# Hydrology-IFH/roger

Hardware: AMD Instinct MI355X
Metric: cell-timesteps/sec on SVAT_benchmark grid (higher is better)
Workload: dtype f64

## Files before the change

roger_amd/build.py:

```python
import os
import subprocess
import sys

PKG = os.path.dirname(os.path.abspath(__file__))
REPO = os.path.dirname(PKG)
CSRC = os.path.join(PKG, "csrc")
LIB = os.path.join(PKG, "libroger_hip.so")
HIPCC = os.environ.get("HIPCC", "/opt/rocm/bin/hipcc")

FLAGS = ["--offload-arch=gfx950", "-O3", "-std=c++17", "-fPIC", "-ffp-contract=off",
         "-I" + os.path.join(REPO, "include"), "-I" + CSRC]


_SAS_DEPS = ("rh_sas_dev.h", "rh_sas_tables.inc", "include/roger_hip_sas.h", "include/rh_sas_arrays.def", "include/roger_hip.h")
UNITS = {
    "roger_hip": ("rh_host.h", "rh_physics.h", "rh_pow.h", "rh_col.h", "rh_sets.inc", "include/roger_hip.h", "include/rh_fields.def",
                  "rh_dev_state.h", "rh_control.h", "rh_step.h", "rh_routing.h", "rh_routing_host.h", "rh_rccl.h"),
    "rh_sas": _SAS_DEPS + ("rh_host.h",),
    "rh_sas_det_iso": _SAS_DEPS + ("rh_sas_kernels.h",),
    "rh_sas_det_anion": _SAS_DEPS + ("rh_sas_kernels.h",),
    "rh_sas_euler_iso": _SAS_DEPS + ("rh_sas_solvers_impl.h",),
    "rh_sas_euler_anion": _SAS_DEPS + ("rh_sas_solvers_impl.h",),
    "rh_sas_rk4_iso": _SAS_DEPS + ("rh_sas_solvers_impl.h",),
    "rh_sas_rk4_anion": _SAS_DEPS + ("rh_sas_solvers_impl.h",),
}
OBJ = os.path.join(PKG, "_obj")


def _newer(target, sources):
    if not os.path.exists(target):
        return True
    t = os.path.getmtime(target)
    return any(os.path.getmtime(s) > t for s in sources)


def _dep_path(d):
    return os.path.join(REPO, d) if d.startswith("include/") else os.path.join(CSRC, d)


def build_native(force=False, verbose=False):
    subprocess.run([sys.executable, os.path.join(REPO, "tools", "gen_sets.py")], check=True)
    os.makedirs(OBJ, exist_ok=True)
    this = os.path.abspath(__file__)
    jobs, objs = [], []
    for unit, deps in UNITS.items():
        src, obj = os.path.join(CSRC, unit + ".hip"), os.path.join(OBJ, unit + ".o")
        objs.append(obj)
        if force or _newer(obj, [src, this] + [_dep_path(d) for d in deps]):
            cmd = [HIPCC] + FLAGS + ["-c", src, "-o", obj]
            if verbose:
                print(" ".join(cmd))
            jobs.append((cmd, subprocess.Popen(cmd)))
    for cmd, job in jobs:
        if job.wait() != 0:
            raise subprocess.CalledProcessError(job.returncode, cmd)
    if force or jobs or _newer(LIB, objs):
        cmd = [HIPCC, "--offload-arch=gfx950", "-shared", "-fPIC"] + objs + ["-o", LIB]
        if verbose:
            print(" ".join(cmd))
        subprocess.run(cmd, check=True)
    return LIB


if __name__ == "__main__":
    print(build_native(force="--force" in sys.argv, verbose=True))
```

roger_amd/csrc/rh_dev_state.h:

```cpp
#ifndef RH_DEV_STATE_H
#define RH_DEV_STATE_H

#define RH_BLOCK 256
#ifndef RH_STRIDE_PAD
#define RH_STRIDE_PAD 0
#endif
#define RH_PRED_BLOCKS 1024
#define RH_DONE_GROUPS 256
#define RH_DONE_STRIDE 32
#define RH_DEVERR_FORCING 1u
#define RH_TAIL_USE_NEXT 1
#define RH_TAIL_CTRL 2
#define RH_TAIL_HOOKS 4
#define RH_TAIL_PRE 16
#define RH_TAIL_SKIP 8
#define RH_SRC_WORD3 0
#ifndef RH_WSTRIDE
#define RH_WSTRIDE 16
#endif
#define RH_SRC_SUMW 1
#ifndef RH_STEP_WAVES
#define RH_STEP_WAVES 2
#endif

struct DevState {
    Consts K;
    rh_scalars S;
    StepCtx X;
    unsigned long long words[4];
    unsigned long long bflags[2][RH_PRED_BLOCKS];
    unsigned long long day_bflags[RH_PRED_BLOCKS];
    int pred_blocks;
    unsigned long long sumw[64 * RH_WSTRIDE];
    unsigned int done_grp[RH_DONE_GROUPS * RH_DONE_STRIDE];
    unsigned int done_top;
    unsigned long long sanity_last;
    unsigned long long pre_words[64];
    int day_cache_ok, day_cache_pad;
    unsigned long long day_fb;
    double day_agg[3];
    unsigned int err_flags;
    rh_scalars S_next;
    StepCtx X_next;
    double *diag;
    long long *diag_steps;
    long long diag_interval;
    int diag_rate, diag_collect, diag_slots;
    int diag_planes[32];
    unsigned long long keep[(RH_NPLANES + 63) / 64];
    int keep_any;
    int *dt_log;
    int dt_log_cap, dt_log_n;
    double forc[3][RH_SLOTS_PER_DAY];
    const double *forc_cell[3];
    double *agg_cell;
    unsigned long long frontw[64 * RH_WSTRIDE], dayw[64 * RH_WSTRIDE], day_word;
    int per_cell;
    const double *series[3];
    const int64_t *calendar[3];
    int64_t nitt_forc;
    long long t_end;
    int skipped;
    int monthly;
    const double *weights[3];
    int n_stations;
    const int *station_idx;
    double *forc_multi;

    const unsigned long long *pmask;

    const double *mlms;
    int64_t mlms_rows;
    int max_slope_per;
    Luts L;
};

struct HostExport {
    rh_scalars S;
    unsigned long long bad, bad_last;
    unsigned int err, pad;
    unsigned long long seq;
};
// ... 163 lines not shown
```

roger_amd/csrc/rh_step.h:

```cpp
#ifndef RH_STEP_H
#define RH_STEP_H

#define LD(name) rh_ld(a, RH_P_##name, i, c.name);
#define ST(name) rh_st(a, RH_P_##name, i, c.name);

constexpr int rh_param_bit(int plane) {
    switch (plane) {
#define RH_PB(name, bit) case RH_P_##name: return bit;
        RH_PARAM_BITS(RH_PB)
#undef RH_PB
        default: return -1;
    }
}
constexpr bool rh_param_derived(int plane) {
    switch (plane) {
#define RH_PD(name) case RH_P_##name:
        RH_DERIVED_FIELDS(RH_PD)
#undef RH_PD
        return true;
        default: return false;
    }
}
#if defined(RH_CENSUS)
#ifndef RH_CENSUS_PMASK
// ... 71 lines not shown
        RH_SEQ_##seq##_LLOAD_##rt(LDP) RH_SEQ_##seq##_ALIAS_##rt(AL) \
    } else {                                                       \
        RH_SEQ_##seq##_LOAD_##rt(LD)                               \
    }
#define RH_DERIVE(rt)                        \
    if constexpr (LAZY) {                    \
        if (um >> 63) rd_##rt(c, K);         \
        rl_##rt(c, K);                       \
    }
#ifdef RH_CENSUS
#define STK(name)
#else
#define STK(name) \
    if ((keepw[RH_P_##name >> 6] >> (RH_P_##name & 63)) & 1ull) rh_st(a, RH_P_##name, i, c.name);
#endif
#define RH_STORES(seq, rt)                                               \
    if constexpr (LAZY && SPARSE) {                                      \
        RH_SEQ_##seq##_SSTORE_##rt(ST)                                   \
        if constexpr (KEEP) { RH_SEQ_##seq##_KSTORE_##rt(STK) }          \
    } else if constexpr (LAZY) {                                         \
        RH_SEQ_##seq##_LSTORE_##rt(ST)                                   \
    } else {                                                             \
        RH_SEQ_##seq##_STORE_##rt(ST) RH_SEQ_##seq##_ROT_##rt(ROT)       \
    }
#define RH_PIN __builtin_amdgcn_sched_barrier(0);
#ifdef RH_STEP_PHASES
__device__ unsigned long long g_step_phases[256 * 64];
#define RH_PH(k)                                                                          \
    if ((threadIdx.x & 63) == 0) {                                                        \
        const unsigned long long t_ = clock64();                                          \
        atomicAdd(&g_step_phases[(blockIdx.x & 255) * 64 + ph_cls * 20 + (k)], t_ - ph_t);                          \
        ph_t = t_;                                                                        \
    }
#else
#define RH_PH(k)
#endif
#define RH_STEP_BODY(seq, mon_rt, MON_LOADS, MON_RUN, sub_rt, sub_call, ne_rt, ne_call, at_rt, at_call) \
    RH_LOADS(seq, rt_select_prec) RH_LOADS(seq, rt_select_pet) MON_LOADS RH_LOADS(seq, rt_interception) RH_PIN  \
    rt_select_prec(c, X, prec_s, ta_s); RH_STORES(seq, rt_select_prec)                                                \
    rt_select_pet(c, X, pet_v, ta_v); RH_STORES(seq, rt_select_pet) RH_PH(1)                                      \
    q = summary_bits_pt(c.prec, c.ta, K);                                                                \
    MON_RUN                                                                                              \
    RH_LOADS(seq, rt_evapotranspiration) RH_PIN                                                                 \
    rt_interception(c, K); RH_STORES(seq, rt_interception) RH_PH(2)                                               \
    RH_LOADS(seq, rt_snow) RH_PIN                                                                               \
    RH_DERIVE(rt_evapotranspiration) rt_evapotranspiration(c, K); RH_STORES(seq, rt_evapotranspiration) RH_PH(3)  \
    RH_LOADS(seq, rt_inf_events) RH_PIN                                                                         \
    rt_snow(c, K, X); RH_STORES(seq, rt_snow) RH_PH(4)                                                            \
    q = summary_bits_sw(q, c.swe, c.swe_top); if (post) post_summary(D, q, dep);                         \
    RH_LOADS(seq, rt_inf_matrix) RH_PIN                                                                         \
    rt_inf_events(c, K, X); RH_STORES(seq, rt_inf_events) RH_PH(5)                                                \
    RH_LOADS(seq, rt_inf_macropores) RH_PIN                                                                     \
    RH_DERIVE(rt_inf_matrix) rt_inf_matrix(c, K, X); RH_STORES(seq, rt_inf_matrix) RH_PH(6)                       \
    RH_LOADS(seq, rt_inf_cracks) RH_PIN                                                                         \
    RH_DERIVE(rt_inf_macropores) rt_inf_macropores(c, K, X); RH_STORES(seq, rt_inf_macropores) RH_PH(7)           \
    RH_LOADS(seq, rt_inf_finish) RH_PIN                                                                         \
    rt_inf_cracks(c, K, X); RH_STORES(seq, rt_inf_cracks) RH_PH(8)                                                \
    RH_LOADS(seq, sub_rt) RH_PIN                                                                                \
    rt_inf_finish(c, K, X); RH_STORES(seq, rt_inf_finish) RH_PH(9)                                                \
    RH_LOADS(seq, rt_capillary_rise) RH_PIN                                                                     \
    RH_DERIVE(sub_rt) sub_call; RH_STORES(seq, sub_rt) RH_PH(10)                                                   \
    RH_LOADS(seq, rt_storage) RH_PIN                                                                            \
    rt_capillary_rise(c, X); RH_STORES(seq, rt_capillary_rise) RH_PH(11)                                           \
    RH_LOADS(seq, ne_rt) RH_PIN                                                                                 \
    RH_DERIVE(rt_storage) rt_storage(c, X); RH_STORES(seq, rt_storage) RH_PH(12)                                   \
    RH_LOADS(seq, at_rt) RH_PIN                                                                                 \
    bad = ne_call; RH_STORES(seq, ne_rt) RH_PH(13)                                                                 \
    at_call; RH_STORES(seq, at_rt) RH_PH(14)

RH_DEV void post_summary(DevState *D, unsigned long long q, unsigned &dep) {
    unsigned long long qq = 0;
#pragma unroll
    for (int b = 0; b <= QB_P_NE0; ++b) qq |= __ballot((q >> b) & 1ull) ? (1ull << b) : 0ull;
    if ((threadIdx.x & 63) == 0 && qq) {
        const unsigned long long old = __hip_atomic_fetch_or(&D->sumw[(blockIdx.x & 63) * RH_WSTRIDE], qq, __ATOMIC_RELAXED, __HIP_MEMORY_SCOPE_AGENT);
        dep |= (unsigned)(old >> 63);
    }
}

template <bool MONTHLY, bool LATERAL, bool LAZY, bool SPARSE, bool KEEP = false, bool MK1 = false>
RH_DEV void step_column(const Arena &a, DevState *D, const StepCtx *Xp, int64_t i, unsigned long long &q, bool &bad, unsigned &dep, unsigned long long um,
                        bool post) {
    {
    const Consts K = D->K;
    const StepCtx X = *Xp;
    Col c;
    double pet_v = X.pet_sel_w, ta_v = X.ta_sel_w;
    double prec_s = X.prec_sel, ta_s = X.ta_sel;
    unsigned long long keepw[(RH_NPLANES + 63) / 64];
#pragma unroll
    for (int k = 0; k < (RH_NPLANES + 63) / 64; ++k) keepw[k] = KEEP ? D->keep[k] : 0ull;
#ifdef RH_STEP_PHASES
    const int ph_cls = X.dt < 0.5 ? 0 : (X.dt < 12 ? 1 : 2);
    unsigned long long ph_t = clock64();
    if ((threadIdx.x & 63) == 0) atomicAdd(&g_step_phases[(blockIdx.x & 255) * 64 + ph_cls * 20 + 19], 1ull);
#endif
#ifndef RH_CENSUS
    if (D->per_cell && X.sel_w >= 0) {
        pet_v = cell_agg(D, a.n, i, 3 * X.sel_w + 2);
        ta_v = cell_agg(D, a.n, i, 3 * X.sel_w + 1);
    }
    if (X.apply_sel == 2 && D->per_cell && X.sel_p >= 0) {
        prec_s = cell_agg(D, a.n, i, 3 * X.sel_p);
        ta_s = cell_agg(D, a.n, i, 3 * X.sel_p + 1);
    }
#endif
    if (MONTHLY && LATERAL) {
        RH_STEP_BODY(step_lateral_monthly, rt_params_surface, RH_LOADS(step_lateral_monthly, rt_params_surface),
                     rt_params_surface(c, D->L, X); RH_STORES(step_lateral_monthly, rt_params_surface),
                     rt_subsurface_runoff_lateral, rt_subsurface_runoff_lateral(c, K, X), rt_num_error_lateral,
                     rt_num_error_lateral(c, K), rt_after_timestep_oned, rt_after_timestep_oned(c))
    } else if (LATERAL) {
        RH_STEP_BODY(step_lateral, , , , rt_subsurface_runoff_lateral, rt_subsurface_runoff_lateral(c, K, X),
                     rt_num_error_lateral, rt_num_error_lateral(c, K), rt_after_timestep_oned, rt_after_timestep_oned(c))
    } else if (MONTHLY) {
        RH_STEP_BODY(step_monthly, rt_params_surface, RH_LOADS(step_monthly, rt_params_surface),
                     rt_params_surface(c, D->L, X); RH_STORES(step_monthly, rt_params_surface), rt_subsurface_runoff,
                     rt_subsurface_runoff(c, X), rt_num_error, rt_num_error(c, K), rt_after_timestep, rt_after_timestep(c))
    } else {
        RH_STEP_BODY(step, , , , rt_subsurface_runoff, rt_subsurface_runoff(c, X), rt_num_error, rt_num_error(c, K),
                     rt_after_timestep, rt_after_timestep(c))
    }
    }
}

template <int MODE, bool LATERAL, bool LAZY, bool SPARSE = false, bool KEEP = false>
__global__ __launch_bounds__(RH_BLOCK, RH_STEP_WAVES) void k_step(Arena a, DevState *D, int flags, int n_groups, int *dst64) {
    const unsigned nb = gridDim.x - ((flags & RH_TAIL_PRE) ? 1u : 0u);
    const bool extra = blockIdx.x >= nb;
    const unsigned x = blockIdx.x & 7u, base_cnt = nb >> 3, rem = nb & 7u;
    const unsigned blk = x * base_cnt + (x < rem ? x : rem) + (blockIdx.x >> 3);
    const int64_t i = extra ? a.n : (int64_t)blk * RH_BLOCK + threadIdx.x;
    __shared__ unsigned wg_done;
    __shared__ CtrlLds tail_lds;
    const StepCtx *Xp = (flags & RH_TAIL_USE_NEXT) ? &D->X_next : &D->X;
#ifndef RH_CENSUS
    const bool halted = Xp->halt != 0;
    if (blockIdx.x == 0 && threadIdx.x == 0) {
        D->skipped = halted ? 1 : 0;
        if (halted) log_dt(D, 0);
    }
    if (halted) return;
#endif
    if (threadIdx.x == 0) wg_done = 0;
    __syncthreads();
    unsigned long long q = 0;
    bool bad = false;
    unsigned dep = 1;
    const bool post = !(flags & RH_TAIL_SKIP);
    if (i < a.n) {
        const bool monthly = MODE == 1 || (MODE == 2 && D->monthly != 0);
        unsigned long long um = 0;
        if constexpr (LAZY) {
#ifdef RH_CENSUS
            um = RH_CENSUS_PMASK;
#else
            const unsigned long long *pm = D->pmask;
            const unsigned long long w = pm ? pm[__builtin_amdgcn_readfirstlane((int)(i >> 6))] : 0ull;
            um = ((unsigned long long)(unsigned)__builtin_amdgcn_readfirstlane((int)(w >> 32)) << 32) | (unsigned)__builtin_amdgcn_readfirstlane((int)w);
#endif
        }
        const bool mk1 = LAZY && ((um >> 62) & 1ull);
#ifdef RH_CENSUS
        if (SPARSE) {
#else
        if (SPARSE && !Xp->last) {
#endif
            if (monthly) step_column<true, LATERAL, LAZY, SPARSE, KEEP>(a, D, Xp, i, q, bad, dep, um, post);
            else if (mk1) step_column<false, LATERAL, LAZY, SPARSE, KEEP, LAZY>(a, D, Xp, i, q, bad, dep, um, post);
            else step_column<false, LATERAL, LAZY, SPARSE, KEEP>(a, D, Xp, i, q, bad, dep, um, post);
        } else {
            if (monthly) step_column<true, LATERAL, LAZY, false>(a, D, Xp, i, q, bad, dep, um, post);
            else step_column<false, LATERAL, LAZY, false>(a, D, Xp, i, q, bad, dep, um, post);
        }
    } else if (post) {
        post_summary(D, 0ull, dep);
    }
#ifndef RH_CENSUS
    if (__builtin_expect(extra && threadIdx.x < 64, 0)) pre_tail(D, tail_lds, flags, dep);
#endif
    const bool any_bad = __any(bad);
    if (!post) {
        if (any_bad && (threadIdx.x & 63) == 0) __hip_atomic_fetch_or(&D->words[2], 1ull, __ATOMIC_RELAXED, __HIP_MEMORY_SCOPE_AGENT);
        return;
    }
    bool last = false;
    if ((threadIdx.x & 63) == 0) {
        if (any_bad) dep |= (unsigned)(__hip_atomic_fetch_or(&D->words[2], 1ull, __ATOMIC_RELAXED, __HIP_MEMORY_SCOPE_AGENT) >> 63);
        const unsigned o = atomicAdd(&wg_done, dep);
        if (o == (RH_BLOCK / 64) - 1) last = grid_completion(D, n_groups);
    }
#ifndef RH_CENSUS
    if (__shfl((int)last, 0)) step_tail(D, tail_lds, flags, dst64);
#endif
}

#ifdef RH_CENSUS
template __global__ void k_step<0, false, true, true>(Arena, DevState *, int, int, int *);
template __global__ void k_step<0, true, true, true>(Arena, DevState *, int, int, int *);
#endif

#define RH_CELL_KERNEL(kname, rt, call)                                       \
    __global__ __launch_bounds__(RH_BLOCK) void kname(Arena a, DevState *D) { \
        const int64_t i = (int64_t)blockIdx.x * RH_BLOCK + threadIdx.x;       \
        if (i >= a.n) return;                                                 \
        const Consts K = D->K;                                                \
        const StepCtx X = D->X;                                               \
        (void)K;                                                              \
        (void)X;                                                              \
        Col c;                                                                \
        RH_SET_LOAD_##rt(LD) call;                                            \
        RH_SET_STORE_##rt(ST)                                                 \
    }

// ... 53 lines not shown
```

roger_amd/csrc/roger_hip.hip:

```cpp
#include <hip/hip_runtime.h>
#include <hip/hip_ext.h>

#include <dlfcn.h>
#include <rccl/rccl.h>

#include <cmath>
#include <cstdio>
#include <cstring>
#include <new>
#include <cstdlib>
#include <string>
#include <type_traits>
#include <utility>
#include <vector>

#include "rh_host.h"
#include "rh_physics.h"
#include "rh_sets.inc"
#include "roger_hip.h"

#include "rh_dev_state.h"
#include "rh_control.h"
#include "rh_step.h"
#include "rh_routing.h"

__global__ __launch_bounds__(RH_BLOCK) void k_max_slope(Arena a, DevState *D) {
    const int64_t i = (int64_t)blockIdx.x * RH_BLOCK + threadIdx.x;
    int v = 0;
    if (i < a.n) rh_ld(a, RH_P_slope_per, i, v);
    for (int off = 32; off; off >>= 1) {
        const int o = __shfl_xor(v, off);
        v = o > v ? o : v;
    }
    if ((threadIdx.x & 63) == 0 && v > 0) atomicMax(&D->max_slope_per, v);
}
RH_CELL_KERNEL(k_topo, rt_topo, rt_topo(c))
RH_CELL_KERNEL(k_params_surface, rt_params_surface, rt_params_surface(c, D->L, X))
RH_CELL_KERNEL(k_params_soil, rt_params_soil, rt_params_soil(c, K, D->L))
// ... 110 lines not shown
    bool pred_daily_stale = true;
    bool front_daily_stale = true;
    int last_front = 0;
};

struct rh_ctx {
    Stream stream;
    rh_config cfg = {};
    int64_t n = 0;
    Arena arena = {};
    DevBuf<char> arena_mem;
    DevBuf<DevState> dev;
    PinnedBlock<HostExport> hexp;
    unsigned long long hexp_seq = 0;
    DevBuf<unsigned long long> pmask_buf;
    int pmask_flags = 7;
    DevBuf<double> forc_cell_buf[3];
    DevBuf<double> weight_buf[3];
    DevBuf<int> station_buf;
    DevBuf<double> forc_multi_buf;
    DevBuf<double> transpose_buf;
    DevBuf<double> agg_cell_buf;
    DevBuf<char> series_buf;
    DevBuf<double> mlms_buf;
    DevBuf<void> stage_buf;
    bool per_cell = false;
    bool forcing_set = false;
    DeviceHolds held;
    bool routed_device_ok = true;
    bool defer_select_ok = true;
    int64_t cell_agg_split_min = 65536;
    bool tail_ok = true;
    int n_groups = 1;
    bool lazy_ok = true;
    bool diag_reads_m1 = false;
    bool sparse_ok = true;
    bool diag_reads_sparse = false;
    int64_t t_end = -1;
    int64_t call_sparse_steps = 0;
    bool cell_front_ok = true;
    int64_t cell_front_max = 2097152;
    DevBuf<double> diag_buf;
    DevBuf<long long> diag_steps_buf;
    long long diag_interval = 86400;
    int diag_n = 0, diag_slots = 0;
    int pred_blocks = 0;
    bool timing = false;
    EventPool events;
    DevBuf<int> dt_log_buf;
    std::vector<double> probe_ms;
    ncclComm_t comm = nullptr;
    bool own_comm = false;
    DevBuf<int> exch_buf;
    int comm_nranks = 1, comm_rank = 0;
    int grid_px = 1, grid_py = 1;
    int planes_held = 0;
    DevBuf<double> route_q;
    DevBuf<int> route_i;
    bool route_halo[2] = {false, false};
    bool route_frame = false;
    bool route_static_done = false;
    std::string err;
};
#define RH_DT_LOG_CAP 65536

static std::string g_create_err;
// ... 96 lines not shown
    ctx->call_sparse_steps += sparse ? 1 : 0;
}
static void fused_step_enqueued(rh_ctx *ctx, int flags, bool lazy, bool sparse, bool exch) {
    ctx->held.rot_consistent = true;
    ctx->held.m1_stale = lazy;
    sparse_step_enqueued(ctx, sparse);
    ctx->held.summary_valid = !(flags & RH_TAIL_SKIP);
    ctx->held.pending_valid = (flags & RH_TAIL_CTRL) != 0;
    ctx->held.pre_valid = (flags & RH_TAIL_PRE) && !(flags & RH_TAIL_CTRL);
    ctx->held.pending_hooks = (flags & RH_TAIL_HOOKS) != 0;
    ctx->held.exch_valid = exch;
}
static void routed_step_enqueued(rh_ctx *ctx, bool sparse) {
    ctx->held.routed_summary = true;
    sparse_step_enqueued(ctx, sparse);
}

#define LAUNCH_CELLS(ctx, kern)                                                                                          \
    do {                                                                                                                 \
        planes_touched(ctx);                                                                                             \
        hipLaunchKernelGGL(kern, dim3(grid_for((ctx)->n)), dim3(RH_BLOCK), 0, (ctx)->stream, (ctx)->arena, (ctx)->dev); \
    } while (0)
#define LAUNCH_PRED(ctx, kern)                                                                                           \
    do {                                                                                                                 \
        planes_touched(ctx);                                                                                             \
        hipLaunchKernelGGL(kern, dim3((ctx)->pred_blocks), dim3(RH_BLOCK), 0, (ctx)->stream, (ctx)->arena, (ctx)->dev, 0); \
    } while (0)
#define LAUNCH_ONE(ctx, kern, ...) hipLaunchKernelGGL(kern, dim3(1), dim3(64), 0, (ctx)->stream, __VA_ARGS__)
#define LAUNCH_WG(ctx, kern, ...) hipLaunchKernelGGL(kern, dim3(1), dim3(RH_BLOCK), 0, (ctx)->stream, __VA_ARGS__)
#define CHECK_LAUNCH(ctx) HIPCHK(ctx, hipGetLastError())

static bool plane_is_stale(const rh_ctx *ctx, int plane) {
    return ctx->held.outputs_stale && pure_output_planes()[ctx->cfg.enable_routing_1D ? 2 : (ctx->cfg.enable_lateral_flow ? 1 : 0)][plane];
}
static int form_param_mask(rh_ctx *ctx, dim3 grid) {
    if (ctx->held.pmask_valid) return RH_OK;
    hipLaunchKernelGGL(k_param_mask, grid, dim3(RH_BLOCK), 0, ctx->stream, ctx->arena, ctx->dev, ctx->pmask_buf, ctx->pmask_flags);
    CHECK_LAUNCH(ctx);
    ctx->held.pmask_valid = true;
    return RH_OK;
}
static int need_forcing(rh_ctx *ctx) {
    if (ctx->forcing_set) return RH_OK;
    return fail(ctx, RH_ERR_STATE, "rh_set_forcing_day / rh_set_forcing_series must be called before the first step");
}
static int need_exch_buf(rh_ctx *ctx) {
    HIPCHK(ctx, ctx->exch_buf.alloc_once(128 * sizeof(int)));
    return RH_OK;
}
static int need_agg_cell_buf(rh_ctx *ctx) {
    if (ctx->agg_cell_buf) return RH_OK;
    HIPCHK(ctx, ctx->agg_cell_buf.alloc(sizeof(double) * 9 * (size_t)ctx->n));
    HIPCHK(ctx, dev_put(ctx, &DevState::agg_cell, *ctx->agg_cell_buf.addr()));
    return RH_OK;
}

#include "rh_rccl.h"

extern "C" {

int rh_abi_version(void) { return RH_ABI_VERSION; }

void rh_default_config(rh_config *cfg) {
    std::memset(cfg, 0, sizeof(*cfg));
    cfg->nx = cfg->ny = 1;
    cfg->pi = 3.14159265358979323846264338327950588;
// ... 138 lines not shown
        static const long long no_limit = -1;
        if ((e = dev_put(ctx, &DevState::t_end, no_limit)) != hipSuccess) return bail(e, "hipMemcpy(t_end)");
    }
    Consts K;
    K.pi = cfg->pi; K.r_mp = cfg->r_mp; K.l_sc = cfg->l_sc; K.sf = cfg->sf; K.ta_fm = cfg->ta_fm; K.rmax = cfg->rmax;
    K.transp_water_stress = cfg->transp_water_stress; K.atol = cfg->atol; K.rtol = cfg->rtol;
    K.clay_min = cfg->clay_min; K.clay_max = cfg->clay_max; K.theta_rew_min = cfg->theta_rew_min;
    K.theta_rew_max = cfg->theta_rew_max; K.rew_min = cfg->rew_min; K.rew_max = cfg->rew_max;
    K.z_evap_max = cfg->z_evap_max; K.zroot_to_zsoil_max = cfg->zroot_to_zsoil_max; K.a_bc = cfg->a_bc; K.b_bc = cfg->b_bc;
    K.end_event = cfg->end_event; K.hpi = cfg->hpi;
    K.dx = cfg->dx; K.lateral = cfg->enable_lateral_flow ? 1 : 0;
    K.dy = cfg->dy; K.routing = cfg->enable_routing_1D ? 1 : 0;
    if ((e = dev_put(ctx, &DevState::K, K)) != hipSuccess) return bail(e, "hipMemcpy(Consts)");
    rh_scalars S;
    std::memset(&S, 0, sizeof(S));
    S.dt = 1;
    S.dt_secs = 3600;
    S.event_id_counter = 1;
    S.year[0] = S.year[1] = 1900;
    S.month[0] = S.month[1] = 1;
    S.doy[0] = S.doy[1] = 1;
    S.sanity_ok = 1;
    if ((e = dev_put(ctx, &DevState::S, S)) != hipSuccess) return bail(e, "hipMemcpy(scalars)");
    if ((e = hipStreamSynchronize(ctx->stream)) != hipSuccess) return bail(e, "hipStreamSynchronize");
    ctx->tail_ok = std::getenv("RH_NO_TAIL_CTRL") == nullptr;
    ctx->routed_device_ok = std::getenv("RH_ROUTED_BY_ROUTINE") == nullptr;
    ctx->defer_select_ok = std::getenv("RH_NO_DEFERRED_SELECT") == nullptr;
    ctx->cell_front_ok = std::getenv("RH_PER_CELL_OLD_FRONT") == nullptr && ctx->defer_select_ok;
    if (const char *v = std::getenv("RH_CELL_FRONT_MAX")) ctx->cell_front_max = std::atoll(v);
    if (const char *v = std::getenv("RH_CELL_AGG_SPLIT_MIN")) ctx->cell_agg_split_min = std::atoll(v);
    ctx->n_groups = (int)((grid_for(ctx->n) + 63) / 64);
    if (ctx->n_groups > RH_DONE_GROUPS) ctx->n_groups = RH_DONE_GROUPS;
    if (ctx->n_groups < 1) ctx->n_groups = 1;
    ctx->pred_blocks = (int)(grid_for(ctx->n) < RH_PRED_BLOCKS ? grid_for(ctx->n) : RH_PRED_BLOCKS);
    if ((e = dev_put(ctx, &DevState::pred_blocks, ctx->pred_blocks)) != hipSuccess) return bail(e, "hipMemcpy(pred_blocks)");
    if ((e = hipStreamSynchronize(ctx->stream)) != hipSuccess) return bail(e, "hipStreamSynchronize");
    hipLaunchKernelGGL(k_init_registry, dim3(grid_for(ctx->n)), dim3(RH_BLOCK), 0, ctx->stream, ctx->arena);
    hipLaunchKernelGGL(k_sync_ctx, dim3(1), dim3(1), 0, ctx->stream, ctx->dev);
    if ((e = hipGetLastError()) != hipSuccess) return bail(e, "kernel launch (is this a gfx950 device?)");
    if ((e = hipStreamSynchronize(ctx->stream)) != hipSuccess) return bail(e, "hipStreamSynchronize");
    *out = ctx;
    return RH_OK;
}

void rh_destroy(rh_ctx *ctx) {
    if (!ctx) return;
    if (ctx->stream) (void)hipStreamSynchronize(ctx->stream);
#ifdef RH_STEP_PHASES
    {
        unsigned long long tp[8];
        if (hipMemcpyFromSymbol(tp, HIP_SYMBOL(g_tail_phases), sizeof(tp)) == hipSuccess && tp[7])
            std::fprintf(stderr, "tail phases: %llu tails, cycles per tail: loads %.0f, hooks+staging %.0f, bits+sums %.0f, decisions %.0f, scalars %.0f, log %.0f; whole tail %.0f\n",
                         tp[7], (double)tp[0] / tp[7], (double)tp[1] / tp[7], (double)tp[2] / tp[7], (double)tp[3] / tp[7], (double)tp[4] / tp[7],
                         (double)tp[5] / tp[7], (double)tp[6] / tp[7]);
        static unsigned long long all[256 * 64];
        unsigned long long h[60] = {0};
        if (hipMemcpyFromSymbol(all, HIP_SYMBOL(g_step_phases), sizeof(all)) == hipSuccess) {
            for (int b = 0; b < 256; ++b)
                for (int k = 0; k < 60; ++k) h[k] += all[b * 64 + k];
            static const char *cls[3] = {"10min", "hourly", "daily"};
            for (int c = 0; c < 3; ++c) {
                if (!h[c * 20 + 19]) continue;
                double tot = 0;
                for (int k = 0; k < 19; ++k) tot += (double)h[c * 20 + k];
                std::fprintf(stderr, "step phases %s: %llu waves, cycles per wave %.0f:", cls[c], h[c * 20 + 19], tot / (double)h[c * 20 + 19]);
                for (int k = 1; k <= 14; ++k) std::fprintf(stderr, " %d:%.1f%%", k, 100.0 * (double)h[c * 20 + k] / tot);
                std::fprintf(stderr, "\n");
            }
        }
    }
#endif
    release_comm(ctx);
    delete ctx;
}

int rh_set_stream(rh_ctx *ctx, void *hip_stream) {
    if (!ctx) return RH_ERR_ARG;
    HIPCHK(ctx, ctx->stream.adopt((hipStream_t)hip_stream));
    return RH_OK;
}

static int device_error(rh_ctx *ctx, unsigned err) {
    if (err & RH_DEVERR_FORCING)
        return fail(ctx, RH_ERR_STATE, "a step began a day beyond the end of the resident forcing series (rh_set_forcing_series): it ran on the "
                                       "previous day's forcing; hand over a longer series (the reference fails on the short slice, "
                                       "benchmarks/SVAT_benchmark.py:151-171)");
    return RH_OK;
}
int rh_sync(rh_ctx *ctx) {
    if (!ctx) return RH_ERR_ARG;
    unsigned err = 0;
    HIPCHK(ctx, hipMemcpyAsync(&err, &ctx->dev->err_flags, sizeof(err), hipMemcpyDeviceToHost, ctx->stream));
    HIPCHK(ctx, hipStreamSynchronize(ctx->stream));
    return device_error(ctx, err);
}

static int plane_bytes(rh_ctx *ctx, int plane, size_t bytes, size_t *elem) {
    if (!ctx) return RH_ERR_ARG;
    if (plane < 0 || plane >= RH_NPLANES) return fail(ctx, RH_ERR_ARG, "unknown plane id");
// ... 212 lines not shown
    else
        LAUNCH_CELLS(ctx, k_core_staged);
    hipLaunchKernelGGL(k_advance, dim3(1), dim3(1), 0, ctx->stream, ctx->dev);
    if (ctx->diag_n) hipLaunchKernelGGL(k_diag, dim3(grid_for(ctx->n)), dim3(RH_BLOCK), 0, ctx->stream, ctx->arena, ctx->dev, 0);
    CHECK_LAUNCH(ctx);
    return RH_OK;
}

int rh_after_timestep(rh_ctx *ctx) {
    if (!ctx) return RH_ERR_ARG;
    if (ctx->cfg.enable_lateral_flow)
        LAUNCH_CELLS(ctx, k_after_timestep_oned);
    else
        LAUNCH_CELLS(ctx, k_after_timestep);
    LAUNCH_ONE(ctx, k_rotate_scalars, ctx->dev);
    CHECK_LAUNCH(ctx);
    return RH_OK;
}

#include "rh_routing_host.h"

static int timing_pair(rh_ctx *ctx, hipEvent_t *ev0, hipEvent_t *ev1) {
    if (!ctx->timing) return RH_OK;
    if (ctx->events.used + 2 > 2 * (size_t)RH_DT_LOG_CAP)
        return fail(ctx, RH_ERR_STATE, "timing: more than 65536 timed steps since rh_enable_timing(1); read the timings and enable again");
    HIPCHK(ctx, ctx->events.next_pair(ev0, ev1));
    return RH_OK;
}

static int launch_fused_kernel(rh_ctx *ctx, int monthly, int flags = 0, int *dst64 = nullptr) {
    hipEvent_t ev0 = nullptr, ev1 = nullptr;
    if (int rc = timing_pair(ctx, &ev0, &ev1)) return rc;
    if (flags & RH_TAIL_CTRL) flags |= RH_TAIL_PRE;
    const dim3 grid(grid_for(ctx->n) + ((flags & RH_TAIL_PRE) ? 1u : 0u)), block(RH_BLOCK);
    const bool lat = ctx->cfg.enable_lateral_flow != 0;
#define RH_LAUNCH_K(K) hipExtLaunchKernelGGL(K, grid, block, 0, ctx->stream, ev0, ev1, 0, ctx->arena, ctx->dev.get(), flags, ctx->n_groups, dst64)
    const bool lazy = ctx->lazy_ok && ctx->held.rot_consistent && !ctx->diag_reads_m1;
    const bool sparse = lazy && ctx->held.sparse_next && monthly < 0;
    const bool keep = sparse && ctx->diag_reads_sparse;
    ctx->held.sparse_next = false;
    if (lazy)
        if (int rc = form_param_mask(ctx, grid)) return rc;
#define RH_LAUNCH_STEP(MODE)                                          \
    do {                                                              \
        if (MODE == 2 && lat && keep)                                 \
            RH_LAUNCH_K((k_step<2, true, true, true, true>));         \
        else if (MODE == 2 && keep)                                   \
            RH_LAUNCH_K((k_step<2, false, true, true, true>));        \
        else if (MODE == 2 && lat && sparse)                          \
            RH_LAUNCH_K((k_step<2, true, true, true>));               \
        else if (MODE == 2 && sparse)                                 \
            RH_LAUNCH_K((k_step<2, false, true, true>));              \
        else if (lat && lazy)                                         \
            RH_LAUNCH_K((k_step<MODE, true, true>));                  \
        else if (lat)                                                 \
            RH_LAUNCH_K((k_step<MODE, true, false>));                 \
        else if (lazy)                                                \
            RH_LAUNCH_K((k_step<MODE, false, true>));                 \
        else                                                          \
            RH_LAUNCH_K((k_step<MODE, false, false>));                \
    } while (0)
    if (monthly < 0) RH_LAUNCH_STEP(2);
    else if (monthly) RH_LAUNCH_STEP(1);
    else RH_LAUNCH_STEP(0);
#undef RH_LAUNCH_STEP
#undef RH_LAUNCH_K
    CHECK_LAUNCH(ctx);
    if (ctx->timing) ctx->events.taken();
    fused_step_enqueued(ctx, flags, lazy, sparse, dst64 != nullptr);
    if (ctx->diag_n) {
        hipLaunchKernelGGL(k_diag, grid, block, 0, ctx->stream, ctx->arena, ctx->dev, 1);
        CHECK_LAUNCH(ctx);
    }
    return RH_OK;
}

static void launch_pred1(rh_ctx *ctx) {
    hipLaunchKernelGGL(k_pred1, dim3(ctx->pred_blocks), dim3(RH_BLOCK), 0, ctx->stream, ctx->arena, ctx->dev, ctx->held.pred_daily_stale ? 1 : 0);
    ctx->held.pred_daily_stale = false;
}
int rh_step_phase1(rh_ctx *ctx) {
    if (!ctx) return RH_ERR_ARG;
    if (int rc = need_forcing(ctx)) return rc;
    planes_touched(ctx);
    front_takes_over(ctx, 1);
    launch_pred1(ctx);
    LAUNCH_WG(ctx, k_reduce, ctx->dev, 0);
    CHECK_LAUNCH(ctx);
    return RH_OK;
}
static void launch_cell_agg(rh_ctx *ctx) {
    const dim3 grid(grid_for(ctx->n)), block(RH_BLOCK);
    const int force = ctx->held.agg_daily_stale ? 1 : 0;
    if (ctx->n >= ctx->cell_agg_split_min) {
        hipLaunchKernelGGL(k_cell_agg<2>, grid, block, 0, ctx->stream, ctx->arena, ctx->dev, force);
        hipLaunchKernelGGL(k_cell_agg<1>, grid, block, 0, ctx->stream, ctx->arena, ctx->dev, force);
    } else
        hipLaunchKernelGGL(k_cell_agg<0>, grid, block, 0, ctx->stream, ctx->arena, ctx->dev, force);
    ctx->held.agg_daily_stale = false;
}
int rh_step_phase2(rh_ctx *ctx) {
    if (!ctx) return RH_ERR_ARG;
    LAUNCH_WG(ctx, k_agg, ctx->dev, 0, 0);
    if (ctx->per_cell) launch_cell_agg(ctx);
// ... 723 lines not shown
```

Before: 5.523 billion.

## Make fused step kernel persistent with occupancy-sized grid and deduplicated summary posts

Changes k_step from one block per 256 cells to a grid sized by occupancy (blocks per CU times CU count), with each block walking several cell blocks in an interleaved stride. Constants, StepCtx and keep words are loaded once per block, and summary-bit atomics are deduplicated across iterations through a posted mask, with the parameter-mask word prefetched for the next iteration. The goal is to cut block launch and scheduling overhead and the repeated per-block atomics and state loads. Also disables machine LICM for the main unit, which may reduce register pressure. The risk is load imbalance or lost latency hiding when fewer blocks are resident.

```diff
diff --git a/roger_amd/build.py b/roger_amd/build.py
--- a/roger_amd/build.py
+++ b/roger_amd/build.py
@@ -24,7 +24,12 @@
     "rh_sas_rk4_iso": _SAS_DEPS + ("rh_sas_solvers_impl.h",),
     "rh_sas_rk4_anion": _SAS_DEPS + ("rh_sas_solvers_impl.h",),
 }
+UNIT_FLAGS = {"roger_hip": ["-mllvm", "-disable-machine-licm"]}
 OBJ = os.path.join(PKG, "_obj")
+
+
+def unit_flags(unit):
+    return FLAGS + UNIT_FLAGS.get(unit, [])
 
 
 def _newer(target, sources):
@@ -47,7 +52,7 @@
         src, obj = os.path.join(CSRC, unit + ".hip"), os.path.join(OBJ, unit + ".o")
         objs.append(obj)
         if force or _newer(obj, [src, this] + [_dep_path(d) for d in deps]):
-            cmd = [HIPCC] + FLAGS + ["-c", src, "-o", obj]
+            cmd = [HIPCC] + unit_flags(unit) + ["-c", src, "-o", obj]
             if verbose:
                 print(" ".join(cmd))
             jobs.append((cmd, subprocess.Popen(cmd)))
diff --git a/roger_amd/csrc/rh_dev_state.h b/roger_amd/csrc/rh_dev_state.h
--- a/roger_amd/csrc/rh_dev_state.h
+++ b/roger_amd/csrc/rh_dev_state.h
@@ -19,6 +19,7 @@
 #define RH_WSTRIDE 16
 #endif
 #define RH_SRC_SUMW 1
+#define RH_KEEP_WORDS ((RH_NPLANES + 63) / 64)
 #ifndef RH_STEP_WAVES
 #define RH_STEP_WAVES 2
 #endif
@@ -47,7 +48,7 @@
     long long diag_interval;
     int diag_rate, diag_collect, diag_slots;
     int diag_planes[32];
-    unsigned long long keep[(RH_NPLANES + 63) / 64];
+    unsigned long long keep[RH_KEEP_WORDS];
     int keep_any;
     int *dt_log;
     int dt_log_cap, dt_log_n;
diff --git a/roger_amd/csrc/rh_step.h b/roger_amd/csrc/rh_step.h
--- a/roger_amd/csrc/rh_step.h
+++ b/roger_amd/csrc/rh_step.h
@@ -127,8 +127,12 @@
         atomicAdd(&g_step_phases[(blockIdx.x & 255) * 64 + ph_cls * 20 + (k)], t_ - ph_t);                          \
         ph_t = t_;                                                                        \
     }
+#define RH_PH_PARAM , unsigned long long &ph_t
+#define RH_PH_ARG , ph_t
 #else
 #define RH_PH(k)
+#define RH_PH_PARAM
+#define RH_PH_ARG
 #endif
 #define RH_STEP_BODY(seq, mon_rt, MON_LOADS, MON_RUN, sub_rt, sub_call, ne_rt, ne_call, at_rt, at_call) \
     RH_LOADS(seq, rt_select_prec) RH_LOADS(seq, rt_select_pet) MON_LOADS RH_LOADS(seq, rt_interception) RH_PIN  \
@@ -142,7 +146,7 @@
     RH_DERIVE(rt_evapotranspiration) rt_evapotranspiration(c, K); RH_STORES(seq, rt_evapotranspiration) RH_PH(3)  \
     RH_LOADS(seq, rt_inf_events) RH_PIN                                                                         \
     rt_snow(c, K, X); RH_STORES(seq, rt_snow) RH_PH(4)                                                            \
-    q = summary_bits_sw(q, c.swe, c.swe_top); if (post) post_summary(D, q, dep);                         \
+    q = summary_bits_sw(q, c.swe, c.swe_top); if (post) post_summary(D, q, dep, posted);                        \
     RH_LOADS(seq, rt_inf_matrix) RH_PIN                                                                         \
     rt_inf_events(c, K, X); RH_STORES(seq, rt_inf_events) RH_PH(5)                                                \
     RH_LOADS(seq, rt_inf_macropores) RH_PIN                                                                     \
@@ -160,42 +164,43 @@
     RH_LOADS(seq, ne_rt) RH_PIN                                                                                 \
     RH_DERIVE(rt_storage) rt_storage(c, X); RH_STORES(seq, rt_storage) RH_PH(12)                                   \
     RH_LOADS(seq, at_rt) RH_PIN                                                                                 \
-    bad = ne_call; RH_STORES(seq, ne_rt) RH_PH(13)                                                                 \
+    bad |= ne_call; RH_STORES(seq, ne_rt) RH_PH(13)                                                                 \
     at_call; RH_STORES(seq, at_rt) RH_PH(14)
 
-RH_DEV void post_summary(DevState *D, unsigned long long q, unsigned &dep) {
+RH_DEV void post_summary(DevState *D, unsigned long long q, unsigned &dep, unsigned long long &posted) {
     unsigned long long qq = 0;
 #pragma unroll
     for (int b = 0; b <= QB_P_NE0; ++b) qq |= __ballot((q >> b) & 1ull) ? (1ull << b) : 0ull;
+    qq &= ~posted;
+    posted |= qq;
     if ((threadIdx.x & 63) == 0 && qq) {
         const unsigned long long old = __hip_atomic_fetch_or(&D->sumw[(blockIdx.x & 63) * RH_WSTRIDE], qq, __ATOMIC_RELAXED, __HIP_MEMORY_SCOPE_AGENT);
         dep |= (unsigned)(old >> 63);
     }
 }
+RH_DEV void post_summary(DevState *D, unsigned long long q, unsigned &dep) {
+    unsigned long long posted = 0;
+    post_summary(D, q, dep, posted);
+}
 
 template <bool MONTHLY, bool LATERAL, bool LAZY, bool SPARSE, bool KEEP = false, bool MK1 = false>
-RH_DEV void step_column(const Arena &a, DevState *D, const StepCtx *Xp, int64_t i, unsigned long long &q, bool &bad, unsigned &dep, unsigned long long um,
-                        bool post) {
+RH_DEV void step_column(const Arena &a, DevState *D, const Consts &K, const StepCtx &X, const unsigned long long (&keepw)[RH_KEEP_WORDS], int64_t i,
+                        unsigned long long &q, bool &bad, unsigned &dep, unsigned long long &posted, unsigned long long um, bool post, bool per_cell RH_PH_PARAM) {
     {
-    const Consts K = D->K;
-    const StepCtx X = *Xp;
     Col c;
     double pet_v = X.pet_sel_w, ta_v = X.ta_sel_w;
     double prec_s = X.prec_sel, ta_s = X.ta_sel;
-    unsigned long long keepw[(RH_NPLANES + 63) / 64];
-#pragma unroll
-    for (int k = 0; k < (RH_NPLANES + 63) / 64; ++k) keepw[k] = KEEP ? D->keep[k] : 0ull;
 #ifdef RH_STEP_PHASES
     const int ph_cls = X.dt < 0.5 ? 0 : (X.dt < 12 ? 1 : 2);
-    unsigned long long ph_t = clock64();
     if ((threadIdx.x & 63) == 0) atomicAdd(&g_step_phases[(blockIdx.x & 255) * 64 + ph_cls * 20 + 19], 1ull);
+    RH_PH(0)
 #endif
 #ifndef RH_CENSUS
-    if (D->per_cell && X.sel_w >= 0) {
+    if (per_cell && X.sel_w >= 0) {
         pet_v = cell_agg(D, a.n, i, 3 * X.sel_w + 2);
         ta_v = cell_agg(D, a.n, i, 3 * X.sel_w + 1);
     }
-    if (X.apply_sel == 2 && D->per_cell && X.sel_p >= 0) {
+    if (X.apply_sel == 2 && per_cell && X.sel_p >= 0) {
         prec_s = cell_agg(D, a.n, i, 3 * X.sel_p);
         ta_s = cell_agg(D, a.n, i, 3 * X.sel_p + 1);
     }
@@ -219,13 +224,25 @@
     }
 }
 
+struct StepWalk {
+    unsigned base, cnt, j0, stride;
+};
+__host__ __device__ inline StepWalk step_walk(unsigned w, unsigned G, unsigned nblk) {
+    if (G < 8u) return StepWalk{0u, nblk, w, G};
+    const unsigned x = w & 7u, base_cnt = nblk >> 3, rem = nblk & 7u;
+    return StepWalk{x * base_cnt + (x < rem ? x : rem), base_cnt + (x < rem ? 1u : 0u), w >> 3, (G >> 3) + (x < (G & 7u) ? 1u : 0u)};
+}
+
 template <int MODE, bool LATERAL, bool LAZY, bool SPARSE = false, bool KEEP = false>
 __global__ __launch_bounds__(RH_BLOCK, RH_STEP_WAVES) void k_step(Arena a, DevState *D, int flags, int n_groups, int *dst64) {
-    const unsigned nb = gridDim.x - ((flags & RH_TAIL_PRE) ? 1u : 0u);
-    const bool extra = blockIdx.x >= nb;
-    const unsigned x = blockIdx.x & 7u, base_cnt = nb >> 3, rem = nb & 7u;
-    const unsigned blk = x * base_cnt + (x < rem ? x : rem) + (blockIdx.x >> 3);
-    const int64_t i = extra ? a.n : (int64_t)blk * RH_BLOCK + threadIdx.x;
+#ifdef RH_STEP_PHASES
+    unsigned long long ph_t = clock64();
+#endif
+    const unsigned G = gridDim.x - ((flags & RH_TAIL_PRE) ? 1u : 0u);
+    const bool extra = blockIdx.x >= G;
+    const unsigned nblk = (unsigned)((a.n + RH_BLOCK - 1) / RH_BLOCK);
+    StepWalk wk = step_walk(blockIdx.x, G, nblk);
+    if (extra) wk.cnt = 0;
     __shared__ unsigned wg_done;
     __shared__ CtrlLds tail_lds;
     const StepCtx *Xp = (flags & RH_TAIL_USE_NEXT) ? &D->X_next : &D->X;
@@ -239,42 +256,60 @@
 #endif
     if (threadIdx.x == 0) wg_done = 0;
     __syncthreads();
-    unsigned long long q = 0;
-    bool bad = false;
+    unsigned long long posted = 0;
+    bool any_bad = false;
     unsigned dep = 1;
     const bool post = !(flags & RH_TAIL_SKIP);
-    if (i < a.n) {
+    if (wk.j0 < wk.cnt) {
+        const Consts K = D->K;
+        const StepCtx X = *Xp;
         const bool monthly = MODE == 1 || (MODE == 2 && D->monthly != 0);
-        unsigned long long um = 0;
-        if constexpr (LAZY) {
+        unsigned long long keepw[RH_KEEP_WORDS];
+#pragma unroll
+        for (int k = 0; k < RH_KEEP_WORDS; ++k) keepw[k] = KEEP ? D->keep[k] : 0ull;
 #ifdef RH_CENSUS
-            um = RH_CENSUS_PMASK;
+        const bool per_cell = false, full = false;
 #else
-            const unsigned long long *pm = D->pmask;
-            const unsigned long long w = pm ? pm[__builtin_amdgcn_readfirstlane((int)(i >> 6))] : 0ull;
-            um = ((unsigned long long)(unsigned)__builtin_amdgcn_readfirstlane((int)(w >> 32)) << 32) | (unsigned)__builtin_amdgcn_readfirstlane((int)w);
-#endif
+        const bool per_cell = D->per_cell != 0;
+        const bool full = X.last != 0;
+        const unsigned long long *pm = LAZY ? D->pmask : nullptr;
+        const int64_t wave0 = (int64_t)(threadIdx.x & ~63u);
+        const auto pm_word = [&](unsigned j) -> unsigned long long {
+            const int64_t c0 = (int64_t)(wk.base + j) * RH_BLOCK + wave0;
+            const unsigned long long w = (pm && j < wk.cnt && c0 < a.n) ? pm[__builtin_amdgcn_readfirstlane((int)(c0 >> 6))] : 0ull;
+            return ((unsigned long long)(unsigned)__builtin_amdgcn_readfirstlane((int)(w >> 32)) << 32) | (unsigned)__builtin_amdgcn_readfirstlane((int)w);
+        };
+        unsigned long long um_next = pm_word(wk.j0);
+#endif
+#ifdef RH_CENSUS
+        {
+            const unsigned j = wk.j0;
+            const unsigned long long um = LAZY ? RH_CENSUS_PMASK : 0ull;
+#else
+        for (unsigned j = wk.j0; j < wk.cnt; j += wk.stride) {
+            const unsigned long long um = um_next;
+            um_next = pm_word(j + wk.stride);
+#endif
+            const int64_t i = (int64_t)(wk.base + j) * RH_BLOCK + threadIdx.x;
+            unsigned long long q = 0;
+            bool bad = false;
+            if (i < a.n) {
+                const bool mk1 = LAZY && ((um >> 62) & 1ull);
+                if (SPARSE && !full) {
+                    if (monthly) step_column<true, LATERAL, LAZY, SPARSE, KEEP>(a, D, K, X, keepw, i, q, bad, dep, posted, um, post, per_cell RH_PH_ARG);
+                    else if (mk1) step_column<false, LATERAL, LAZY, SPARSE, KEEP, LAZY>(a, D, K, X, keepw, i, q, bad, dep, posted, um, post, per_cell RH_PH_ARG);
+                    else step_column<false, LATERAL, LAZY, SPARSE, KEEP>(a, D, K, X, keepw, i, q, bad, dep, posted, um, post, per_cell RH_PH_ARG);
+                } else {
+                    if (monthly) step_column<true, LATERAL, LAZY, false>(a, D, K, X, keepw, i, q, bad, dep, posted, um, post, per_cell RH_PH_ARG);
+                    else step_column<false, LATERAL, LAZY, false>(a, D, K, X, keepw, i, q, bad, dep, posted, um, post, per_cell RH_PH_ARG);
+                }
+            }
+            any_bad = any_bad || __any(bad);
         }
-        const bool mk1 = LAZY && ((um >> 62) & 1ull);
-#ifdef RH_CENSUS
-        if (SPARSE) {
-#else
-        if (SPARSE && !Xp->last) {
-#endif
-            if (monthly) step_column<true, LATERAL, LAZY, SPARSE, KEEP>(a, D, Xp, i, q, bad, dep, um, post);
-            else if (mk1) step_column<false, LATERAL, LAZY, SPARSE, KEEP, LAZY>(a, D, Xp, i, q, bad, dep, um, post);
-            else step_column<false, LATERAL, LAZY, SPARSE, KEEP>(a, D, Xp, i, q, bad, dep, um, post);
-        } else {
-            if (monthly) step_column<true, LATERAL, LAZY, false>(a, D, Xp, i, q, bad, dep, um, post);
-            else step_column<false, LATERAL, LAZY, false>(a, D, Xp, i, q, bad, dep, um, post);
-        }
-    } else if (post) {
-        post_summary(D, 0ull, dep);
     }
 #ifndef RH_CENSUS
     if (__builtin_expect(extra && threadIdx.x < 64, 0)) pre_tail(D, tail_lds, flags, dep);
 #endif
-    const bool any_bad = __any(bad);
     if (!post) {
         if (any_bad && (threadIdx.x & 63) == 0) __hip_atomic_fetch_or(&D->words[2], 1ull, __ATOMIC_RELAXED, __HIP_MEMORY_SCOPE_AGENT);
         return;
diff --git a/roger_amd/csrc/roger_hip.hip b/roger_amd/csrc/roger_hip.hip
--- a/roger_amd/csrc/roger_hip.hip
+++ b/roger_amd/csrc/roger_hip.hip
@@ -4,6 +4,7 @@
 #include <dlfcn.h>
 #include <rccl/rccl.h>
 
+#include <cassert>
 #include <cmath>
 #include <cstdio>
 #include <cstring>
@@ -180,6 +181,8 @@
     int64_t cell_agg_split_min = 65536;
     bool tail_ok = true;
     int n_groups = 1;
+    unsigned step_slots = 0;
+    int step_groups = 1;
     bool lazy_ok = true;
     bool diag_reads_m1 = false;
     bool sparse_ok = true;
@@ -342,6 +345,17 @@
 
 static bool plane_is_stale(const rh_ctx *ctx, int plane) {
     return ctx->held.outputs_stale && pure_output_planes()[ctx->cfg.enable_routing_1D ? 2 : (ctx->cfg.enable_lateral_flow ? 1 : 0)][plane];
+}
+[[maybe_unused]] static bool step_walk_covers(unsigned g, unsigned nblk) {
+    std::vector<unsigned char> taken(nblk, 0);
+    for (unsigned w = 0; w < g; ++w) {
+        const StepWalk wk = step_walk(w, g, nblk);
+        for (unsigned j = wk.j0; j < wk.cnt; j += wk.stride)
+            if (wk.base + j >= nblk || taken[wk.base + j]++) return false;
+    }
+    for (unsigned b = 0; b < nblk; ++b)
+        if (!taken[b]) return false;
+    return true;
 }
 static int form_param_mask(rh_ctx *ctx, dim3 grid) {
     if (ctx->held.pmask_valid) return RH_OK;
@@ -546,6 +560,23 @@
     ctx->n_groups = (int)((grid_for(ctx->n) + 63) / 64);
     if (ctx->n_groups > RH_DONE_GROUPS) ctx->n_groups = RH_DONE_GROUPS;
     if (ctx->n_groups < 1) ctx->n_groups = 1;
+    {
+        const unsigned blocks = grid_for(ctx->n);
+        long long slots = -1;
+        if (const char *v = std::getenv("RH_STEP_SLOTS")) slots = std::atoll(v);
+        if (slots < 0) {
+            int per_cu = 0, cus = 0;
+            if ((e = hipOccupancyMaxActiveBlocksPerMultiprocessor(&per_cu, k_step<2, false, true, true>, RH_BLOCK, 0)) != hipSuccess)
+                return bail(e, "hipOccupancyMaxActiveBlocksPerMultiprocessor(k_step)");
+            if ((e = hipDeviceGetAttribute(&cus, hipDeviceAttributeMultiprocessorCount, cfg->device)) != hipSuccess)
+                return bail(e, "hipDeviceGetAttribute(multiprocessor count)");
+            slots = (long long)per_cu * cus;
+        }
+        ctx->step_slots = (slots == 0 || slots > (long long)blocks) ? blocks : (unsigned)slots;
+        assert(step_walk_covers(ctx->step_slots, blocks));
+        ctx->step_groups = (int)((ctx->step_slots + 63) / 64);
+        if (ctx->step_groups > RH_DONE_GROUPS) ctx->step_groups = RH_DONE_GROUPS;
+    }
     ctx->pred_blocks = (int)(grid_for(ctx->n) < RH_PRED_BLOCKS ? grid_for(ctx->n) : RH_PRED_BLOCKS);
     if ((e = dev_put(ctx, &DevState::pred_blocks, ctx->pred_blocks)) != hipSuccess) return bail(e, "hipMemcpy(pred_blocks)");
     if ((e = hipStreamSynchronize(ctx->stream)) != hipSuccess) return bail(e, "hipStreamSynchronize");
@@ -578,7 +609,7 @@
                 double tot = 0;
                 for (int k = 0; k < 19; ++k) tot += (double)h[c * 20 + k];
                 std::fprintf(stderr, "step phases %s: %llu waves, cycles per wave %.0f:", cls[c], h[c * 20 + 19], tot / (double)h[c * 20 + 19]);
-                for (int k = 1; k <= 14; ++k) std::fprintf(stderr, " %d:%.1f%%", k, 100.0 * (double)h[c * 20 + k] / tot);
+                for (int k = 0; k <= 14; ++k) std::fprintf(stderr, " %d:%.1f%%", k, 100.0 * (double)h[c * 20 + k] / tot);
                 std::fprintf(stderr, "\n");
             }
         }
@@ -857,15 +888,15 @@
     hipEvent_t ev0 = nullptr, ev1 = nullptr;
     if (int rc = timing_pair(ctx, &ev0, &ev1)) return rc;
     if (flags & RH_TAIL_CTRL) flags |= RH_TAIL_PRE;
-    const dim3 grid(grid_for(ctx->n) + ((flags & RH_TAIL_PRE) ? 1u : 0u)), block(RH_BLOCK);
+    const dim3 grid(ctx->step_slots + ((flags & RH_TAIL_PRE) ? 1u : 0u)), block(RH_BLOCK);
     const bool lat = ctx->cfg.enable_lateral_flow != 0;
-#define RH_LAUNCH_K(K) hipExtLaunchKernelGGL(K, grid, block, 0, ctx->stream, ev0, ev1, 0, ctx->arena, ctx->dev.get(), flags, ctx->n_groups, dst64)
+#define RH_LAUNCH_K(K) hipExtLaunchKernelGGL(K, grid, block, 0, ctx->stream, ev0, ev1, 0, ctx->arena, ctx->dev.get(), flags, ctx->step_groups, dst64)
     const bool lazy = ctx->lazy_ok && ctx->held.rot_consistent && !ctx->diag_reads_m1;
     const bool sparse = lazy && ctx->held.sparse_next && monthly < 0;
     const bool keep = sparse && ctx->diag_reads_sparse;
     ctx->held.sparse_next = false;
     if (lazy)
-        if (int rc = form_param_mask(ctx, grid)) return rc;
+        if (int rc = form_param_mask(ctx, dim3(grid_for(ctx->n)))) return rc;
 #define RH_LAUNCH_STEP(MODE)                                          \
     do {                                                              \
         if (MODE == 2 && lat && keep)                                 \
@@ -894,7 +925,7 @@
     if (ctx->timing) ctx->events.taken();
     fused_step_enqueued(ctx, flags, lazy, sparse, dst64 != nullptr);
     if (ctx->diag_n) {
-        hipLaunchKernelGGL(k_diag, grid, block, 0, ctx->stream, ctx->arena, ctx->dev, 1);
+        hipLaunchKernelGGL(k_diag, dim3(grid_for(ctx->n)), block, 0, ctx->stream, ctx->arena, ctx->dev, 1);
         CHECK_LAUNCH(ctx);
     }
     return RH_OK;
```

Result: no change. 5.508 billion (median of 5 runs) (-0.3%).
